# kan-bayashi/espnet

Hardware: AMD Instinct MI355X
Metric: frames/sec, 12L Conformer hybrid CTC/attention training step (B=32 T=1000 d=256 per GPU) (higher is better)
Workload: dtype f32

## Files before the change

### espnet_amd/_lib.py

```python
import ctypes as C
import os

import torch

_HERE = os.path.dirname(os.path.abspath(__file__))
LIB_PATH = os.path.join(_HERE, "csrc", "libespnet_amd_hip.so")


class EamdError(RuntimeError):
    pass


class GatherT(C.Structure):
    _fields_ = [("enabled", C.c_int32), ("C", C.c_int32), ("ntap", C.c_int32), ("Ho", C.c_int32),
                ("Wo", C.c_int32), ("Hin", C.c_int32), ("Win", C.c_int32), ("sh", C.c_int32),
                ("sw", C.c_int32), ("dh", C.c_int32 * 9), ("dw", C.c_int32 * 9)]


class RowMapT(C.Structure):
    _fields_ = [("enabled", C.c_int32), ("Ho", C.c_int32), ("Wo", C.c_int32), ("Hc", C.c_int32),
                ("Wc", C.c_int32), ("sh", C.c_int32), ("oh", C.c_int32), ("sw", C.c_int32),
                ("ow", C.c_int32)]


class RowStatsT(C.Structure):
    _fields_ = [("part", C.c_void_p), ("col", C.c_void_p), ("zcol", C.c_void_p), ("zfix", C.c_void_p),
                ("fix", C.c_int32), ("reserved", C.c_int32),
                ("rowc", C.c_void_p), ("gscale", C.c_void_p), ("scale", C.c_float), ("reserved2", C.c_int32)]


class GemmT(C.Structure):
    _fields_ = [("A", C.c_void_p), ("B", C.c_void_p), ("C", C.c_void_p), ("bias", C.c_void_p),
                ("aux", C.c_void_p), ("R", C.c_void_p), ("colsum", C.c_void_p),
                ("M", C.c_int32), ("N", C.c_int32), ("K", C.c_int32),
                ("transA", C.c_int32), ("transB", C.c_int32),
                ("lda", C.c_int64), ("ldb", C.c_int64), ("ldc", C.c_int64), ("ldaux", C.c_int64),
                ("ldr", C.c_int64),
                ("batch1", C.c_int32), ("batch2", C.c_int32),
                ("sA1", C.c_int64), ("sA2", C.c_int64), ("sB1", C.c_int64), ("sB2", C.c_int64),
                ("sC1", C.c_int64), ("sC2", C.c_int64),
                ("alpha", C.c_float), ("beta", C.c_float),
                ("a_act", C.c_int32), ("b_act", C.c_int32), ("epilogue", C.c_int32),
                ("splitk", C.c_int32), ("precision", C.c_int32), ("tile", C.c_int32),
                ("gather", GatherT), ("cmap", RowMapT),
                ("Cb", C.c_void_p), ("in_dtype", C.c_int32), ("aux_dtype", C.c_int32),
                ("drop_p", C.c_float), ("drop_salt", C.c_uint64), ("drop_step", C.c_void_p), ("Hb", C.c_void_p),
                ("h_act", C.c_int32),
                ("a_drop_p", C.c_float), ("b_drop_p", C.c_float), ("a_drop_salt", C.c_uint64), ("b_drop_salt", C.c_uint64),
                ("h_dtype", C.c_int32),
                ("stats", RowStatsT)]


class FfnT(C.Structure):
    _fields_ = [("x", C.c_void_p), ("w1", C.c_void_p), ("b1", C.c_void_p), ("w2", C.c_void_p), ("b2", C.c_void_p),
                ("R", C.c_void_p), ("out", C.c_void_p), ("f", C.c_void_p), ("h", C.c_void_p),
                ("M", C.c_int32), ("D", C.c_int32), ("F", C.c_int32), ("act", C.c_int32),
                ("alpha", C.c_float), ("p_in", C.c_float), ("salt_in", C.c_uint64), ("p_out", C.c_float),
                ("salt_out", C.c_uint64), ("drop_step", C.c_void_p), ("dtype", C.c_int32), ("hsplit", C.c_int32),
                ("ln_x", C.c_void_p), ("ln_w", C.c_void_p), ("ln_b", C.c_void_p), ("ln_mean", C.c_void_p),
                ("ln_rstd", C.c_void_p), ("ln_eps", C.c_float), ("reserved2", C.c_int32),
                ("lnb_x", C.c_void_p), ("lnb_gamma", C.c_void_p), ("lnb_mean", C.c_void_p), ("lnb_rstd", C.c_void_p),
                ("lnb_dres", C.c_void_p), ("lnb_ws", C.c_void_p), ("lnb_drop_out", C.c_void_p), ("lnb_drop_salt", C.c_uint64),
                ("lnb_drop_p", C.c_float), ("reserved3", C.c_int32)]


class RowProjT(C.Structure):
    _fields_ = [("a", C.c_void_p), ("lda", C.c_int64), ("w", C.c_void_p), ("bias", C.c_void_p), ("R", C.c_void_p),
                ("ldr", C.c_int64), ("out", C.c_void_p), ("ldo", C.c_int64),
                ("M", C.c_int32), ("K", C.c_int32), ("N", C.c_int32), ("a_act", C.c_int32),
                ("alpha", C.c_float), ("p_out", C.c_float), ("salt_out", C.c_uint64), ("drop_step", C.c_void_p),
                ("ln_x", C.c_void_p), ("ln_w", C.c_void_p), ("ln_b", C.c_void_p), ("ln_mean", C.c_void_p),
                ("ln_rstd", C.c_void_p), ("ln_eps", C.c_float), ("lnb_drop_p", C.c_float),
                ("a_scale", C.c_void_p), ("a_shift", C.c_void_p), ("a_out", C.c_void_p),
                ("lnb_x", C.c_void_p), ("lnb_gamma", C.c_void_p), ("lnb_mean", C.c_void_p), ("lnb_rstd", C.c_void_p),
                ("lnb_dres", C.c_void_p), ("lnb_ws", C.c_void_p), ("lnb_drop_out", C.c_void_p), ("lnb_drop_salt", C.c_uint64)]


class FfnPackT(C.Structure):
    _fields_ = [("w1", C.c_void_p), ("w2", C.c_void_p), ("fwd_first", C.c_void_p), ("fwd_second", C.c_void_p),
                ("bwd_first", C.c_void_p), ("bwd_second", C.c_void_p), ("D", C.c_int32), ("F", C.c_int32)]


class RowProjPackT(C.Structure):
    _fields_ = [("w", C.c_void_p), ("image", C.c_void_p), ("K", C.c_int32), ("N", C.c_int32), ("ldw", C.c_int32),
                ("trans", C.c_int32)]


class LstmSeqFwdT(C.Structure):
    _fields_ = [("gx", C.c_void_p), ("w_hh", C.c_void_p), ("b_hh", C.c_void_p), ("live", C.c_void_p),
                ("h_out", C.c_void_p), ("c_out", C.c_void_p), ("y", C.c_void_p), ("acts", C.c_void_p),
                ("reverse", C.c_int32), ("reserved", C.c_int32)]


class LstmSeqBwdT(C.Structure):
    _fields_ = [("dy", C.c_void_p), ("w_t", C.c_void_p), ("acts", C.c_void_p), ("c_out", C.c_void_p),
                ("live", C.c_void_p), ("dgates", C.c_void_p), ("reverse", C.c_int32), ("reserved", C.c_int32)]


_lib = None

SYMBOLS = [
    "eamd_abi_version", "eamd_gemm", "eamd_gemm_multi", "eamd_gemm_group_plan", "eamd_gemm_group_launch", "eamd_ffn_fwd", "eamd_ffn_bwd", "eamd_ffn_pack_f32", "eamd_ffn_pack_bf16", "eamd_ffn_pack_f32_multi", "eamd_rowproj", "eamd_rowproj_pack_f32", "eamd_rowproj_lnb_workspace", "eamd_layernorm_fwd", "eamd_layernorm_bwd_workspace", "eamd_layernorm_bwd_drop_f32", "eamd_layernorm_bwd", "eamd_layernorm_bwd_reduce", "eamd_attn_fwd", "eamd_attn_bwd_q", "eamd_attn_fwd_f32", "eamd_attn_bwd_q_f32", "eamd_attn_bwd_kv_f32", "eamd_attn_bwd_kv", "eamd_softmax_fwd",
    "eamd_softmax_bwd", "eamd_lsm_loss", "eamd_argmax_rows", "eamd_reduce_sum", "eamd_log_softmax_rows", "eamd_transducer_expand_rows", "eamd_topk_rows", "eamd_topk_rows_i32", "eamd_weighted_topk_rows", "eamd_beam_step", "eamd_beam_step_dyn", "eamd_decode_self_attn_dyn", "eamd_beam_slots_dyn", "eamd_ctc_prefix_psi_dyn", "eamd_ctc_prefix_state_dyn", "eamd_embed_pe_dyn", "eamd_copy_jobs", "eamd_embed_pe_ld", "eamd_linear_rows_f32", "eamd_linear_rows_ln_f32", "eamd_decode_self_attn", "eamd_beam_slots", "eamd_decode_src_attn", "eamd_decode_src_attn_group", "eamd_decode_src_attn_split", "eamd_decode_src_attn_split_workspace", "eamd_weighted_sum", "eamd_beam_select", "eamd_beam_finish",
    "eamd_axpby", "eamd_cast_bf16", "eamd_scale_dev", "eamd_act_fwd", "eamd_act_bwd", "eamd_glu_fwd", "eamd_glu_bwd",
    "eamd_add_bias2", "eamd_add_cast_bf16", "eamd_add_block_f32", "eamd_add_cast_colsum2", "eamd_add_colsum2_f32", "eamd_colsum", "eamd_embed_pe", "eamd_embed_bwd", "eamd_posenc", "eamd_posenc_scaled", "eamd_posenc_scaled_bwd", "eamd_permute4",
    "eamd_dropout", "eamd_rng_advance", "eamd_dwconv_fwd", "eamd_dwconv_glu_fwd", "eamd_dwconv_glu_bwd_x", "eamd_dwconv_glu_bwd_w", "eamd_dwconv_bwd_x", "eamd_dwconv_bwd_w", "eamd_bn_nslab",
    "eamd_bn_stats", "eamd_bn_finalize", "eamd_bn_apply", "eamd_bn_bwd", "eamd_bn_stats_bounded", "eamd_bn_bwd_bounded", "eamd_mask_time", "eamd_conv1_fwd", "eamd_conv1_bwd_w_workspace", "eamd_conv1_bwd_w",
    "eamd_conv2_weight_prep", "eamd_conv2_weight_grad", "eamd_add_sos_eos", "eamd_ctc_collapse",
    "eamd_ctc_workspace_bytes", "eamd_ctc_loss", "eamd_ctc_prefix_score", "eamd_ctc_prefix_score_batch", "eamd_ctc_prefix_psi", "eamd_ctc_prefix_state", "eamd_grad_norm", "eamd_sched_step", "eamd_adam_step", "eamd_adadelta_step", "eamd_add_gradient_noise",
    "eamd_specaug", "eamd_global_mvn", "eamd_utterance_mvn", "eamd_reflect_pad", "eamd_logmel", "eamd_unfold1d", "eamd_fold1d", "eamd_attloc_convmax_fwd", "eamd_attloc_convmax_bwd", "eamd_layernorm_bwd_drop",
    "eamd_lstm_cell_fwd", "eamd_lstm_cell_bwd", "eamd_lstm_step_fwd", "eamd_lstm_step_bwd", "eamd_lstm_seq_sync_bytes", "eamd_lstm_seq_fwd", "eamd_lstm_seq_bwd", "eamd_lstm_seq_status", "eamd_lstm_seq_status_merge", "eamd_gru_cell_fwd", "eamd_gru_cell_bwd", "eamd_maxpool2x2_fwd", "eamd_maxpool2x2_bwd", "eamd_mask_rows",
    "eamd_joint_fwd", "eamd_joint_bwd", "eamd_rnnt_workspace", "eamd_rnnt_loss", "eamd_rnnt_grad", "eamd_rnnt_node_stats", "eamd_rnnt_node_stats_part", "eamd_rnnt_row_coef", "eamd_rnnt_alpha_beta", "eamd_rnnt_node_grad",
    "eamd_conv3x3_c1_fwd", "eamd_conv3x3_c1_bwd_w_workspace", "eamd_conv3x3_c1_bwd_w", "eamd_attloc_fwd", "eamd_attloc_bwd_energy", "eamd_attloc_bwd_workspace", "eamd_attloc_bwd_energy_conv", "eamd_attloc_bwd_conv",
    "eamd_att_dot_energy_fwd", "eamd_att_dot_energy_bwd", "eamd_att_ctx_fwd", "eamd_att_ctx_bwd",
]


def lib():
    global _lib
    if _lib is None:
        if not os.path.exists(LIB_PATH):
            raise EamdError(
                f"{LIB_PATH} not found: build it with `python -c 'import __graft_entry__ as g; g.build()'` "
                "or `make -C espnet_amd/csrc` (there is no CPU fallback)")
        _lib = C.CDLL(LIB_PATH)
        _lib.eamd_ctc_workspace_bytes.restype = C.c_int64
        _lib.eamd_layernorm_bwd_workspace.restype = C.c_int64
        _lib.eamd_rnnt_workspace.restype = C.c_int64
        _lib.eamd_attloc_bwd_workspace.restype = C.c_int64
        _lib.eamd_conv1_bwd_w_workspace.restype = C.c_int64
        _lib.eamd_lstm_seq_sync_bytes.restype = C.c_int64
        _lib.eamd_conv3x3_c1_bwd_w_workspace.restype = C.c_int64
        for s in SYMBOLS:
            getattr(_lib, s)
    return _lib


_raw_stream = getattr(torch._C, "_cuda_getCurrentRawStream", None)
_cur_device = getattr(torch._C, "_cuda_getDevice", None)


def stream_ptr():
    if _raw_stream is not None and _cur_device is not None:
        return C.c_void_p(_raw_stream(_cur_device()))
    return C.c_void_p(torch.cuda.current_stream().cuda_stream)


EAMD_EUNSUPPORTED = -2


def check(rc, what):
    if rc != 0:
        raise EamdError(f"{what} failed with code {rc}")


def ptr(t, offset=0):
    if t is None:
        return None
    if not t.is_cuda:
        raise EamdError("espnet_amd kernels need GPU tensors (no CPU fallback in the product path)")
    if offset == 0:
        return C.c_void_p(t.data_ptr())
    return C.c_void_p(t.data_ptr() + offset * t.element_size())


def f32(t):
    if t.dtype != torch.float32:
        raise EamdError(f"expected float32 tensor, got {t.dtype}")
    return t
```

### espnet_amd/functional.py

```python
import math

import torch

from . import ops
from .ops import (ACT_NONE, ACT_RELU, ACT_SWISH, EPI_DACT_FACTOR, EPI_MUL_AUX, EPI_MUL_DSWISH, EPI_MUL_RELU_MASK, EPI_NONE,
                  EPI_RELU)


class GradSink:

    on_done = None
    on_use = None

    @staticmethod
    def use(params):
        if GradSink.on_use is not None and torch.is_grad_enabled():
            GradSink.on_use(params)
        return params

    def __init__(self, params):
        self.params = list(params)
        self.ret = [None] * len(self.params)

    def buf(self, i):
# ... 876 lines not shown
        gl = d = bmean = None
        nbt = getattr(running_mean, "_eamd_nbt", None)
        if FUSE_GLU_DWCONV:
            d = ops.dwconv_glu_fwd(a, wd.view(Cc, K), bd_, B, T, Cc, K,
                                   bn=(bn_eps, bn_momentum, running_mean, running_var, nbt) if (training and bound is None) else None)
            if d is not None and training and bound is None:
                d, bmean, brstd = d
        if d is None:
            gl = ops.glu_fwd(a, Cc)
            d = ops.dwconv_fwd(gl, wd.view(Cc, K), bd_, B, T, Cc, K)
        if training:
            if bmean is None:
                bmean, brstd = ops.bn_stats(d, M, Cc, bn_eps, bn_momentum, running_mean, running_var, nbt, bound=bound)
        else:
            bmean = running_mean
            brstd = ops.axpby(running_var, None, 1.0, 0.0)
            brstd = torch.rsqrt_(brstd.add_(bn_eps))
        e = ops.bn_apply(d, bmean, brstd, g, be, M, Cc, act, adt)
        ctx.rp = rp
        if rp is not None:
            out = ops.rowproj(e, rp[2], Cc, bias=b2, R=x2, drop=(p_out, s_out) if p_out > 0.0 else None)
        elif p_out > 0.0 and (ops.fast() or ops.f32_epilogue_drop()):
            out = ops.linear_fwd(e, ops.wshadow(w2).view(Cc, Cc), b2, R=x2, drop=(p_out, s_out))
        elif p_out > 0.0:
            br = ops.linear_fwd(e, ops.wshadow(w2).view(Cc, Cc), b2)
            out = ops.axpby(x2, ops.dropout(br, p_out, s_out), 1.0, 1.0)
        else:
            out = ops.linear_fwd(e, ops.wshadow(w2).view(Cc, Cc), b2, R=x2 if eps is not None else None)
        ctx.save_for_backward(x2, mean, rstd, xn, a, gl, d, bmean, brstd, e)
        ctx.pr = GradSink.use(params)
        ctx.cfg = (B, T, D, Cc, K, act, training, drop)
        ctx.bound = bound
        ctx.prev = _prev_drop(x)
        return _tag_out(out.view(B, T, D), p_out, s_out)

    @staticmethod
    def backward(ctx, dout):
        x2, mean, rstd, xn, a, gl, d, bmean, brstd, e = ctx.saved_tensors
        ln_w, ln_b, w1, b1, wd, bd_, g, be, w2, b2 = ctx.pr
        B, T, D, Cc, K, act, training, (p_out, s_out) = ctx.cfg
        M = B * T
        adt = ops.act_dtype()
        sink = GradSink(ctx.pr)
        do = dout.reshape(M, D).contiguous()
        dob, g_drop = _grad_operand(dout, do, p_out, s_out)
        rp = ctx.rp if g_drop is None else None
        ops.linear_bwd_w(dob, e, sink.buf(8).view(Cc, Cc), db=sink.buf(9), a_drop=g_drop)
        if rp is not None:
            de = ops.rowproj(dob, rp[3], Cc)
        else:
            de = ops.linear_bwd_x(dob, ops.wshadow(w2).view(Cc, Cc), a_drop=g_drop)
        dd = ops.bn_bwd(de, d, bmean, brstd, g, be, sink.buf(6), sink.buf(7), M, Cc, act, training, bound=ctx.bound)
        if gl is None:
            da = ops.dwconv_glu_bwd_x(dd, wd.view(Cc, K), a, B, T, Cc, K, adt)
            if ctx.bound is not None:
                ops.mask_time(da, T, ctx.bound[1])
            ops.dwconv_glu_bwd_w(dd, a, sink.buf(4).view(Cc, K), sink.buf(5), B, T, Cc, K)
        else:
            dgl = ops.dwconv_bwd_x(dd, wd.view(Cc, K), B, T, Cc, K)
            ops.dwconv_bwd_w(dd, gl, sink.buf(4).view(Cc, K), sink.buf(5), B, T, Cc, K)
            da = ops.glu_bwd(dgl, a, Cc, adt)
            if ctx.bound is not None:
                ops.mask_time(da, T, ctx.bound[1])
        ops.linear_bwd_w(da, xn, sink.buf(2).view(2 * Cc, D), db=sink.buf(3))
        if rp is not None and da.dtype == torch.float32:
            dx = _rp_ln_bwd(da, rp[1], x2, ln_w, mean, rstd, do, sink.buf(0), sink.buf(1), ctx.prev, (B, T, D))
        else:
            dxn = ops.linear_bwd_x(da, ops.wshadow(w1).view(2 * Cc, D))
            dx = _ln_bwd_out(dxn, x2, ln_w, mean, rstd, do, sink.buf(0), sink.buf(1), ctx.prev, (B, T, D))
        return (dx, None, None, None, None, None, None, None, None) + sink.results()


_TAPS_FWD = [(kh, kw) for kh in range(3) for kw in range(3)]
_CLASSES = [((0, 0), [(0, 0), (0, 2), (2, 0), (2, 2)]), ((0, 1), [(0, 1), (2, 1)]),
            ((1, 0), [(1, 0), (1, 2)]), ((1, 1), [(1, 1)])]


def _conv3s2_fwd(y_in, w, b, B, Hi, Wi, Cc, adt):
    Ho, Wo = (Hi - 3) // 2 + 1, (Wi - 3) // 2 + 1
    wf, wd = ops.conv2_weight_prep(w, adt)
    g = ops.make_gather(Cc, _TAPS_FWD, Ho, Wo, Hi, Wi, 2, 2)
    M = B * Ho * Wo
    y = torch.empty(M, Cc, device=y_in.device, dtype=adt)
    ops.gemm(y_in, wf, y, M, Cc, 9 * Cc, 9 * Cc, Cc, Cc, transB=1, bias=b, epilogue=EPI_RELU, gather=g)
    return y, wd, Ho, Wo


def _conv3s2_bwd(dy, y_in, wd, dw_buf, db_buf, B, Hi, Wi, Ho, Wo, Cc, adt):
    dev = dy.device
    M = B * Ho * Wo
    ops.colsum(dy, db_buf)
    dwf = torch.zeros(9 * Cc, Cc, device=dev, dtype=torch.float32)
    g = ops.make_gather(Cc, _TAPS_FWD, Ho, Wo, Hi, Wi, 2, 2)
    f32_big = (not ops.fast()) and Cc % 128 == 0
    tile = 128 if f32_big else 64
    ntile = (9 * Cc // tile) * ((Cc + tile - 1) // tile)
    want = 1024 if ops.fast() else 1008 if f32_big else 2304
    sk = max(2, min(64, (want + ntile - 1) // ntile, max(1, M // 256)))
    ops.gemm(y_in, dy, dwf, 9 * Cc, Cc, M, 9 * Cc, Cc, Cc, transA=1, transB=1, gather=g, splitk=sk, tile=tile)
    ops.conv2_weight_grad(dwf, dw_buf, Cc, Cc)
    dy_in = torch.empty(y_in.shape, device=dev, dtype=adt)
    q0, classes = 0, []
    for (ph, pw), taps in _CLASSES:
        Hc, Wc = (Hi - ph + 1) // 2, (Wi - pw + 1) // 2
        if Hc > 0 and Wc > 0:
            gt = ops.make_gather(Cc, [((ph - kh) // 2, (pw - kw) // 2) for kh, kw in taps], Hc, Wc, Ho, Wo, 1, 1)
            cm = ops.make_rowmap(Hc, Wc, Hi, Wi, 2, ph, 2, pw)
            nt = len(taps)
            ops.gemm(dy, wd, dy_in, B * Hc * Wc, Cc, nt * Cc, nt * Cc, Cc, Cc, transB=1, b_off=q0 * Cc * Cc,
                     gather=gt, cmap=cm, epilogue=EPI_MUL_RELU_MASK, aux=y_in, ldaux=Cc, defer=classes)
        q0 += len(taps)
    ops.gemm_multi(classes)
    return dy_in


def _taps(k):
    return [(kh, kw) for kh in range(k) for kw in range(k)]


def _conv_ks_fwd(y_in, w, b, B, Hi, Wi, Cc, adt, k, st):
    Ho, Wo = (Hi - k) // st + 1, (Wi - k) // st + 1
    KK = k * k
    wf = torch.empty(KK, Cc, Cc, device=y_in.device, dtype=torch.float32)
    ops.permute4(w.contiguous(), wf, (Cc, Cc, KK, 1), (1, Cc, Cc * Cc, 0))
    wd = torch.empty(KK, Cc, Cc, device=y_in.device, dtype=torch.float32)
    ops.permute4(w.contiguous(), wd, (Cc, Cc, KK, 1), (Cc, 1, Cc * Cc, 0))
    wf, wd = ops.to_act(wf), ops.to_act(wd)
    M = B * Ho * Wo
    y32 = torch.empty(M, Cc, device=y_in.device, dtype=torch.float32)
    taps = _taps(k)
    for t0 in range(0, KK, 9):
        ch = taps[t0:t0 + 9]
        g = ops.make_gather(Cc, ch, Ho, Wo, Hi, Wi, st, st)
        ops.gemm(y_in, wf, y32, M, Cc, len(ch) * Cc, len(ch) * Cc, Cc, Cc, transB=1, bias=b if t0 == 0 else None,
                 beta=0.0 if t0 == 0 else 1.0, gather=g, b_off=t0 * Cc * Cc)
    y = ops.dropout(y32, 0.0, 0, act=ACT_RELU, out_dtype=adt)
    return y, wd, Ho, Wo


def _conv_ks_bwd(dy, y_in, wd, dw_buf, db_buf, B, Hi, Wi, Ho, Wo, Cc, adt, k, st):
    dev = dy.device
    M = B * Ho * Wo
    KK = k * k
    taps = _taps(k)
    ops.colsum(dy, db_buf)
    dwf = torch.zeros(KK * Cc, Cc, device=dev, dtype=torch.float32)
    for t0 in range(0, KK, 9):
        ch = taps[t0:t0 + 9]
        g = ops.make_gather(Cc, ch, Ho, Wo, Hi, Wi, st, st)
        ntile = (len(ch) * Cc // 64) * ((Cc + 63) // 64)
        sk = max(2, min(64, (1024 + ntile - 1) // ntile, max(1, M // 256)))
        ops.gemm(y_in, dy, dwf, len(ch) * Cc, Cc, M, len(ch) * Cc, Cc, Cc, transA=1, transB=1, gather=g, splitk=sk, tile=64,
                 c_off=t0 * Cc * Cc)
    ops.permute4(dwf, dw_buf, (KK, Cc, Cc, 1), (1, KK, Cc * KK, 0), accumulate=True)
    dy_in = torch.empty(y_in.shape, device=dev, dtype=adt)
    order, classes = [], []
    for ph in range(st):
        for pw in range(st):
            ct = [(kh, kw) for kh in range(ph, k, st) for kw in range(pw, k, st)]
            classes.append(((ph, pw), ct))
            order += [kh * k + kw for kh, kw in ct]
    wd_cls = wd.index_select(0, torch.tensor(order, device=dev)).contiguous()
    q0, jobs = 0, []
    for (ph, pw), ct in classes:
        Hc, Wc = (Hi - ph + st - 1) // st, (Wi - pw + st - 1) // st
        if Hc > 0 and Wc > 0 and ct:
            gt = ops.make_gather(Cc, [((ph - kh) // st, (pw - kw) // st) for kh, kw in ct], Hc, Wc, Ho, Wo, 1, 1)
            cm = ops.make_rowmap(Hc, Wc, Hi, Wi, st, ph, st, pw)
            nt = len(ct)
            ops.gemm(dy, wd_cls, dy_in, B * Hc * Wc, Cc, nt * Cc, nt * Cc, Cc, Cc, transB=1, b_off=q0 * Cc * Cc,
                     gather=gt, cmap=cm, epilogue=EPI_MUL_RELU_MASK, aux=y_in, ldaux=Cc, defer=jobs)
        q0 += len(ct)
    ops.gemm_multi(jobs)
    return dy_in


class Conv2dSubsamplingFn(torch.autograd.Function):

    @staticmethod
    def forward(ctx, x, xscale, c1_w, c1_b, lin_w, lin_b, *convs):
        B, T, F = x.shape
        Cc = c1_w.shape[0]
        D = lin_w.shape[0]
        H1, W1 = (T - 3) // 2 + 1, (F - 3) // 2 + 1
# ... 174 lines not shown
```

### espnet_amd/ops.py

```python
import ctypes as C
import os
import math

import torch

from . import _lib
from ._lib import GatherT, GemmT, RowMapT, check, ptr, stream_ptr

ACT_NONE, ACT_RELU, ACT_SWISH = 0, 1, 2
EPI_NONE, EPI_RELU, EPI_SWISH, EPI_MUL_RELU_MASK, EPI_MUL_DSWISH, EPI_MUL_AUX, EPI_DACT_FACTOR, EPI_ROW_STATS, EPI_ROW_GRAD = 0, 1, 2, 3, 4, 5, 6, 7, 8

_PRECISIONS = {"fp32": 0, "bf16": 1}
_state = {"precision": 0}


def set_precision(name):
    if name not in _PRECISIONS:
        raise ValueError(f"precision must be one of {list(_PRECISIONS)}")
    _state["precision"] = _PRECISIONS[name]


def get_precision():
    return [k for k, v in _PRECISIONS.items() if v == _state["precision"]][0]

# ... 1450 lines not shown

def dwconv_glu_bwd_x(dy, w, a, B, T, Cc, K, out_dtype=torch.float32):
    da = torch.empty(a.shape, device=a.device, dtype=out_dtype)
    check(_lib.lib().eamd_dwconv_glu_bwd_x(ptr(dy), ptr(w), ptr(a), ptr(da), int(out_dtype == torch.bfloat16), B, T, Cc, K,
                                           stream_ptr()), "eamd_dwconv_glu_bwd_x")
    return da


def dwconv_glu_bwd_w(dy, a, dw, db, B, T, Cc, K):
    assert dw.numel() == Cc * K and (db is None or db.numel() == Cc)
    check(_lib.lib().eamd_dwconv_glu_bwd_w(ptr(dy), ptr(a), ptr(dw), ptr(db), B, T, Cc, K, stream_ptr()),
          "eamd_dwconv_glu_bwd_w")


def bn_stats(x, M, Cc, eps, momentum, running_mean, running_var, num_batches_tracked=None, bound=None):
    nslab = _lib.lib().eamd_bn_nslab(C.c_int64(M), Cc)
    ws = torch.empty(3 * Cc * nslab, device=x.device, dtype=torch.float32)
    mean = torch.empty(Cc, device=x.device, dtype=torch.float32)
    rstd = torch.empty(Cc, device=x.device, dtype=torch.float32)
    assert num_batches_tracked is None or (num_batches_tracked.dtype == torch.int64 and num_batches_tracked.is_cuda)
    if bound is not None:
        check(_lib.lib().eamd_bn_stats_bounded(ptr(x), ptr(ws), ptr(mean), ptr(rstd), ptr(running_mean), ptr(running_var),
                                               ptr(num_batches_tracked), C.c_int64(M), Cc, C.c_float(eps), C.c_float(momentum),
                                               int(bound[0]), ptr(bound[1]), stream_ptr()), "eamd_bn_stats_bounded")
        return mean, rstd
    check(_lib.lib().eamd_bn_stats(ptr(x), ptr(ws), ptr(mean), ptr(rstd), ptr(running_mean), ptr(running_var),
                                   ptr(num_batches_tracked), C.c_int64(M), Cc, C.c_float(eps), C.c_float(momentum), stream_ptr()),
          "eamd_bn_stats")
    return mean, rstd


def bn_apply(x, mean, rstd, gamma, beta, M, Cc, act, out_dtype=torch.float32):
    y = torch.empty(x.shape, device=x.device, dtype=out_dtype)
    check(_lib.lib().eamd_bn_apply(ptr(x), ptr(mean), ptr(rstd), ptr(gamma), ptr(beta), ptr(y), C.c_int64(M), Cc,
                                   act, 1 if out_dtype == torch.bfloat16 else 0, stream_ptr()), "eamd_bn_apply")
    return y


def bn_bwd(dy, x, mean, rstd, gamma, beta, dgamma, dbeta, M, Cc, act, training, bound=None):
    nslab = _lib.lib().eamd_bn_nslab(C.c_int64(M), Cc)
    ws = torch.empty((2 * nslab + 2) * Cc, device=x.device, dtype=torch.float32)
    dx = torch.empty_like(x)
    if bound is not None:
        check(_lib.lib().eamd_bn_bwd_bounded(ptr(dy), ptr(x), ptr(mean), ptr(rstd), ptr(gamma), ptr(beta), ptr(ws), ptr(dx),
                                             ptr(dgamma), ptr(dbeta), C.c_int64(M), Cc, act, int(training), int(bound[0]),
                                             ptr(bound[1]), stream_ptr()), "eamd_bn_bwd_bounded")
        return dx
    check(_lib.lib().eamd_bn_bwd(ptr(dy), ptr(x), ptr(mean), ptr(rstd), ptr(gamma), ptr(beta), ptr(ws), ptr(dx),
                                 ptr(dgamma), ptr(dbeta), C.c_int64(M), Cc, act, int(training), stream_ptr()),
          "eamd_bn_bwd")
    return dx


def conv1_fwd(x, w, bias, B, T, F, Cc, out_dtype=torch.float32):
    H, W = (T - 3) // 2 + 1, (F - 3) // 2 + 1
    assert x.numel() == B * T * F and w.numel() == Cc * 9
    y = torch.empty(B, H, W, Cc, device=x.device, dtype=out_dtype)
    check(_lib.lib().eamd_conv1_fwd(ptr(x), ptr(w), ptr(bias), ptr(y), B, T, F, Cc,
                                    1 if out_dtype == torch.bfloat16 else 0, stream_ptr()), "eamd_conv1_fwd")
    return y


def conv1_bwd_w(dy, x, dw, db, B, T, F, Cc):
    L = _lib.lib()
    ws = torch.empty(int(L.eamd_conv1_bwd_w_workspace(B, T, Cc)), device=x.device, dtype=torch.float32)
    check(L.eamd_conv1_bwd_w(ptr(dy), ptr(x), ptr(dw), ptr(db), ptr(ws), B, T, F, Cc,
                             1 if dy.dtype == torch.bfloat16 else 0, stream_ptr()), "eamd_conv1_bwd_w")


def conv2_weight_prep(w, out_dtype=torch.float32):
    Co, Ci = w.shape[0], w.shape[1]
    wf = torch.empty(9, Ci, Co, device=w.device, dtype=out_dtype)
    wd = torch.empty(9, Co, Ci, device=w.device, dtype=out_dtype)
    check(_lib.lib().eamd_conv2_weight_prep(ptr(w), ptr(wf), ptr(wd), Co, Ci,
                                            1 if out_dtype == torch.bfloat16 else 0, stream_ptr()),
          "eamd_conv2_weight_prep")
    return wf, wd


def conv2_weight_grad(dwf, dw, Co, Ci):
    check(_lib.lib().eamd_conv2_weight_grad(ptr(dwf), ptr(dw), Co, Ci, stream_ptr()), "eamd_conv2_weight_grad")


def permute4(src, dst, dims, dst_strides, accumulate=False):
    d0, d1, d2, d3 = dims
    s0, s1, s2, s3 = dst_strides
    assert src.numel() == d0 * d1 * d2 * d3
    assert (d0 - 1) * s0 + (d1 - 1) * s1 + (d2 - 1) * s2 + (d3 - 1) * s3 < dst.numel()
    check(_lib.lib().eamd_permute4(ptr(src), ptr(dst), d0, d1, d2, d3, C.c_int64(s0), C.c_int64(s1), C.c_int64(s2),
                                   C.c_int64(s3), int(accumulate), stream_ptr()), "eamd_permute4")


def add_sos_eos(ys_pad, sos, eos, ignore_id):
    B, L = ys_pad.shape
    assert ys_pad.dtype == torch.int64 and ys_pad.is_contiguous()
    ys_in = torch.empty(B, L + 1, device=ys_pad.device, dtype=torch.int64)
    ys_out = torch.empty(B, L + 1, device=ys_pad.device, dtype=torch.int64)
    olen = torch.empty(B, device=ys_pad.device, dtype=torch.int32)
    check(_lib.lib().eamd_add_sos_eos(ptr(ys_pad), ptr(ys_in), ptr(ys_out), ptr(olen), B, L, sos, eos, ignore_id,
                                      stream_ptr()), "eamd_add_sos_eos")
    return ys_in, ys_out, olen


def ctc_collapse(ids, hlens, blank):
    B, T = ids.shape
    assert ids.dtype == torch.int32 and ids.is_contiguous()
    out = torch.empty(B, T, device=ids.device, dtype=torch.int32)
    outlen = torch.empty(B, device=ids.device, dtype=torch.int32)
    check(_lib.lib().eamd_ctc_collapse(ptr(ids), ptr(hlens), ptr(out), ptr(outlen), B, T, blank, stream_ptr()),
          "eamd_ctc_collapse")
    return out, outlen


def ctc_loss(acts_btv, ys_pad, ilens, blank=0, ignore_id=-1, grad_scale=1.0, want_grad=True, time_major=False):
    if time_major:
        T, B, V = acts_btv.shape
        st, sb = B * V, V
    else:
        B, T, V = acts_btv.shape
        st, sb = V, T * V
    L = ys_pad.shape[1]
    assert acts_btv.is_contiguous() and ys_pad.is_contiguous() and ys_pad.dtype == torch.int64
    assert ilens.dtype == torch.int32 and ilens.numel() == B and ys_pad.shape[0] == B
    ws_bytes = _lib.lib().eamd_ctc_workspace_bytes(B, T, L)
    ws = torch.empty(ws_bytes, device=acts_btv.device, dtype=torch.uint8)
    nll = torch.empty(B, device=acts_btv.device, dtype=torch.float32)
    grad = torch.empty_like(acts_btv) if want_grad else None
    check(_lib.lib().eamd_ctc_loss(ptr(acts_btv), C.c_int64(st), C.c_int64(sb), ptr(ys_pad), ptr(ilens), ptr(nll),
                                   ptr(grad), C.c_int64(st), C.c_int64(sb), ptr(ws), B, T, V, L, blank, ignore_id,
                                   C.c_float(grad_scale), stream_ptr()), "eamd_ctc_loss")
    return nll, grad


def ctc_prefix_score(logp, r_prev, cand, last, olen, blank, eos):
    T, V = logp.shape
    nhyp, ncand = cand.shape
    assert r_prev.shape == (nhyp, T, 2) and cand.dtype == torch.int32 and logp.is_contiguous()
    psi = torch.empty(nhyp, ncand, device=logp.device, dtype=torch.float32)
    r_new = torch.empty(nhyp, ncand, T, 2, device=logp.device, dtype=torch.float32)
    check(_lib.lib().eamd_ctc_prefix_score(ptr(logp), ptr(r_prev.contiguous()), ptr(cand.contiguous()), ptr(last),
                                           ptr(olen), ptr(psi), ptr(r_new), nhyp, ncand, T, V, blank, eos,
                                           stream_ptr()), "eamd_ctc_prefix_score")
    return psi, r_new


def ctc_prefix_score_batch(logp, lens, per_utt, r_prev, cand, last, olen, blank, eos):
    U, Tmax, V = logp.shape
    nhyp, ncand = cand.shape
    assert nhyp == U * per_utt and r_prev.shape == (nhyp, Tmax, 2) and cand.dtype == torch.int32 and logp.is_contiguous()
    assert lens.dtype == torch.int32 and lens.numel() == U
    psi = torch.empty(nhyp, ncand, device=logp.device, dtype=torch.float32)
    r_new = torch.zeros(nhyp, ncand, Tmax, 2, device=logp.device, dtype=torch.float32)
    check(_lib.lib().eamd_ctc_prefix_score_batch(ptr(logp), ptr(lens), U, per_utt, ptr(r_prev.contiguous()), ptr(cand.contiguous()),
                                                 ptr(last), ptr(olen), ptr(psi), ptr(r_new), ncand, Tmax, V, blank, eos,
                                                 stream_ptr()), "eamd_ctc_prefix_score_batch")
    return psi, r_new


def ctc_prefix_psi(logp, lens, per_utt, r_prev, cand, last, olen, blank, eos, olen_dev=None):
    U, Tmax, V = logp.shape
    nhyp, ncand = cand.shape
    assert nhyp == U * per_utt and r_prev.shape == (nhyp, Tmax, 2) and cand.dtype == torch.int32 and logp.is_contiguous()
    psi = torch.empty(nhyp, ncand, device=logp.device, dtype=torch.float32)
    rc = _lib.lib().eamd_ctc_prefix_psi_dyn(ptr(logp), ptr(lens), U, per_utt, ptr(r_prev.contiguous()), ptr(cand.contiguous()), ptr(last),
                                            int(olen), ptr(olen_dev), ptr(psi), ncand, Tmax, V, blank, eos, stream_ptr())
    if rc == _lib.EAMD_EUNSUPPORTED:
# ... 608 lines not shown
```

### include/espnet_amd.h

```cpp
#ifndef ESPNET_AMD_H_
#define ESPNET_AMD_H_
#include <stdint.h>
#ifdef __cplusplus
extern "C" {
#endif

int eamd_abi_version(void);

typedef struct {
  int32_t enabled;
  int32_t C;
  int32_t ntap;
  int32_t Ho, Wo;
  int32_t Hin, Win;
  int32_t sh, sw;
  int32_t dh[9], dw[9];
} eamd_gather_t;

typedef struct {
  int32_t enabled;
  int32_t Ho, Wo;
  int32_t Hc, Wc;
  int32_t sh, oh, sw, ow;
} eamd_rowmap_t;
// ... 332 lines not shown
int eamd_lstm_seq_bwd(const eamd_lstm_seq_bwd_t* jobs, int njobs, int T, int B, int H, void* sync_ws, void* stream);
int eamd_lstm_seq_status(const void* sync_ws, void* stream);
int eamd_lstm_seq_status_merge(const void* sync_ws, void* sticky, void* stream);
int eamd_gru_cell_fwd(const float* gx, const float* gh, const float* h_prev, const uint8_t* live, float* h, float* y,
                      float* acts, int B, int H, void* stream);
int eamd_gru_cell_bwd(const float* dy, const float* dh, const float* acts, const float* h_prev, const uint8_t* live,
                      float* dgx, float* dgh, float* dh_direct, int B, int H, void* stream);
int eamd_maxpool2x2_fwd(const float* x, float* y, uint8_t* idx, int B, int H, int W, int C, void* stream);
int eamd_maxpool2x2_bwd(const float* dy, const uint8_t* idx, float* dx, int B, int H, int W, int C, void* stream);
int eamd_mask_rows(const float* x, const uint8_t* keep, float* y, int64_t rows, int D, void* stream);
int eamd_unfold1d(const void* x, void* col, int B, int T, int C, int k, int bf16, void* stream);
int eamd_fold1d(const float* dcol, float* dx, int B, int T, int C, int k, void* stream);
int eamd_conv3x3_c1_fwd(const float* x, const float* w, const float* bias, void* y, int B, int T, int F, int C,
                        int y_bf16, void* stream);
int64_t eamd_conv3x3_c1_bwd_w_workspace(int B, int T, int C);
int eamd_conv3x3_c1_bwd_w(const void* dy, const float* x, float* dw, float* db, float* workspace, int B, int T, int F,
                          int C, int dy_bf16, void* stream);
int eamd_attloc_fwd(const float* att_prev, const float* conv_w, const float* w_att, const float* pre_enc,
                    const float* dec_proj, const float* gvec, const float* gb, const int32_t* lens, const float* enc_h,
                    float scaling, float* e, float* th, float* conv, float* w, float* ctx, int B, int T, int A, int C,
                    int K, int R, int E, void* stream);
int eamd_attloc_bwd_energy(const float* dctx, const float* dw_ext, const float* w, const float* enc_h, const float* th,
                           const float* gvec, float scaling, float* de, float* d_enc_h, float* df, float* dgvec,
                           float* dgb, float* d_dec_proj, int B, int T, int A, int E, void* stream);
int64_t eamd_attloc_bwd_workspace(int B, int T, int A, int C);
int eamd_attloc_bwd_energy_conv(const float* dctx, const float* dw_ext, const float* w, const float* enc_h, const float* th,
                                const float* gvec, float scaling, const float* conv, const float* w_att, float* de,
                                float* d_enc_h, float* df, float* dconv, float* dgvec, float* dgb, float* d_dec_proj,
                                float* dw_att, float* workspace, int accumulate, int B, int T, int A, int C, int E,
                                void* stream);
int eamd_att_dot_energy_fwd(const float* k, const float* q, const int32_t* lens, float* e, int B, int T, int A,
                            void* stream);
int eamd_att_dot_energy_bwd(const float* de, const float* k, const float* q, float* dk, float* dq, int B, int T, int A,
                            void* stream);
int eamd_att_ctx_fwd(const float* e, const float* v, float scaling, float* w, float* ctx, int B, int T, int E,
                     void* stream);
int eamd_att_ctx_bwd(const float* dctx, const float* dw_ext, const float* w, const float* v, float scaling, float* de,
                     float* d_v, float* dsum, int B, int T, int E, void* stream);
int eamd_attloc_bwd_conv(const float* dconv, const float* conv_w, const float* att_prev, float* d_prev, float* dconv_w,
                         int B, int T, int C, int K, int R, void* stream);
int eamd_attloc_convmax_fwd(const float* att_prev, const float* conv_w, float* pooled, int32_t* idx, int B, int T, int C,
                            int K, void* stream);
int eamd_attloc_convmax_bwd(const float* dpool, const float* pooled, const int32_t* idx, const float* att_prev,
                            const float* conv_w, float* d_prev, float* dconv_w, int B, int T, int C, int K, void* stream);

int eamd_joint_fwd(const float* enc, const float* dec, float* out, void* out_bf16, int B, int T, int U, int J, int act,
                   void* stream);
int eamd_joint_bwd(const float* dh, const float* enc, const float* dec, float* d_enc, float* d_dec, int B, int T, int U,
                   int J, int act, void* stream);
int64_t eamd_rnnt_workspace(int B, int T, int U);
int eamd_rnnt_loss(const float* logits, const int32_t* labels, const int32_t* tlens, const int32_t* ulens,
                   float* workspace, float* loss, float* grad, int B, int T, int U, int V, int blank,
                   const float* gscale_dev, float scale, void* stream);
int eamd_rnnt_grad(const float* logits, const int32_t* labels, const int32_t* tlens, const int32_t* ulens,
                   const float* workspace, float* grad, int B, int T, int U, int V, int blank, const float* gscale_dev,
                   float scale, void* stream);
int eamd_rnnt_node_stats(const float* logits_rows, const int32_t* labels, float* workspace, int64_t node0, int64_t nrows,
                         int B, int T, int U, int V, int blank, void* stream);
int eamd_rnnt_alpha_beta(float* workspace, const int32_t* tlens, const int32_t* ulens, float* loss, int B, int T, int U,
                         void* stream);
int eamd_rnnt_node_stats_part(const float* part, const float* zlab, const float* zblank, float* workspace, int64_t node0,
                              int64_t nrows, int tiles_n, int B, int T, int U, void* stream);
int eamd_rnnt_row_coef(const int32_t* labels, const int32_t* tlens, const int32_t* ulens, const float* workspace, float* rowc,
                       int32_t* col, int64_t node0, int64_t nrows, int B, int T, int U, void* stream);
int eamd_rnnt_node_grad(const float* logits_rows, float* grad_rows, void* grad_rows_bf16, const int32_t* labels,
                        const int32_t* tlens, const int32_t* ulens, const float* workspace, int64_t node0, int64_t nrows,
                        int B, int T, int U, int V, int blank, const float* gscale_dev, float scale, void* stream);

int eamd_grad_norm(const float* g, int64_t n, float* workspace, float* gnorm_out, void* stream);
int eamd_sched_step(float* state, const float* gnorm, int mode, float base_lr, float factor, float dmodel,
                    float warmup, float beta1, float beta2, float max_norm, void* stream);
int eamd_adam_step(float* p, const float* g, float* m, float* v, void* p_bf16, int64_t n, const float* state,
                   float beta1, float beta2, float eps, float weight_decay, void* stream);
int eamd_adadelta_step(float* p, const float* g, float* square_avg, float* acc_delta, void* p_bf16, int64_t n,
                       const float* state, float rho, float weight_decay, void* stream);
int eamd_add_gradient_noise(float* g, int64_t n, float sigma, const uint64_t* step_dev, uint64_t salt, void* stream);

int eamd_add_sos_eos(const int64_t* ys_pad, int64_t* ys_in, int64_t* ys_out, int32_t* olen, int B, int L, int sos,
                     int eos, int ignore_id, void* stream);
int eamd_ctc_collapse(const int32_t* ids, const int32_t* hlens, int32_t* out, int32_t* outlen, int B, int T,
                      int blank, void* stream);
int eamd_conv2_weight_prep(const float* w, void* wf, void* wd, int Co, int Ci, int out_bf16, void* stream);
int eamd_conv2_weight_grad(const float* dwf, float* dw, int Co, int Ci, void* stream);

#ifdef __cplusplus
}
#endif
#endif
```

Before: 1.125 million.

## Add dedicated f32 MFMA kernels for stride-2 3x3 subsampling conv fwd and dx

```diff
diff --git a/espnet_amd/_lib.py b/espnet_amd/_lib.py
--- a/espnet_amd/_lib.py
+++ b/espnet_amd/_lib.py
@@ -106,7 +106,7 @@
     "eamd_add_bias2", "eamd_add_cast_bf16", "eamd_add_block_f32", "eamd_add_cast_colsum2", "eamd_add_colsum2_f32", "eamd_colsum", "eamd_embed_pe", "eamd_embed_bwd", "eamd_posenc", "eamd_posenc_scaled", "eamd_posenc_scaled_bwd", "eamd_permute4",
     "eamd_dropout", "eamd_rng_advance", "eamd_dwconv_fwd", "eamd_dwconv_glu_fwd", "eamd_dwconv_glu_bwd_x", "eamd_dwconv_glu_bwd_w", "eamd_dwconv_bwd_x", "eamd_dwconv_bwd_w", "eamd_bn_nslab",
     "eamd_bn_stats", "eamd_bn_finalize", "eamd_bn_apply", "eamd_bn_bwd", "eamd_bn_stats_bounded", "eamd_bn_bwd_bounded", "eamd_mask_time", "eamd_conv1_fwd", "eamd_conv1_bwd_w_workspace", "eamd_conv1_bwd_w",
-    "eamd_conv2_weight_prep", "eamd_conv2_weight_grad", "eamd_add_sos_eos", "eamd_ctc_collapse",
+    "eamd_conv2_weight_prep", "eamd_conv2_weight_grad", "eamd_conv3s2_f32_fwd", "eamd_conv3s2_f32_bwd_x", "eamd_add_sos_eos", "eamd_ctc_collapse",
     "eamd_ctc_workspace_bytes", "eamd_ctc_loss", "eamd_ctc_prefix_score", "eamd_ctc_prefix_score_batch", "eamd_ctc_prefix_psi", "eamd_ctc_prefix_state", "eamd_grad_norm", "eamd_sched_step", "eamd_adam_step", "eamd_adadelta_step", "eamd_add_gradient_noise",
     "eamd_specaug", "eamd_global_mvn", "eamd_utterance_mvn", "eamd_reflect_pad", "eamd_logmel", "eamd_unfold1d", "eamd_fold1d", "eamd_attloc_convmax_fwd", "eamd_attloc_convmax_bwd", "eamd_layernorm_bwd_drop",
     "eamd_lstm_cell_fwd", "eamd_lstm_cell_bwd", "eamd_lstm_step_fwd", "eamd_lstm_step_bwd", "eamd_lstm_seq_sync_bytes", "eamd_lstm_seq_fwd", "eamd_lstm_seq_bwd", "eamd_lstm_seq_status", "eamd_lstm_seq_status_merge", "eamd_gru_cell_fwd", "eamd_gru_cell_bwd", "eamd_maxpool2x2_fwd", "eamd_maxpool2x2_bwd", "eamd_mask_rows",
diff --git a/espnet_amd/csrc/conv3s2_f32.hip b/espnet_amd/csrc/conv3s2_f32.hip
--- /dev/null
+++ b/espnet_amd/csrc/conv3s2_f32.hip
@@ -0,0 +1,310 @@
+#include "common.h"
+#include "../../include/espnet_amd.h"
+
+namespace {
+
+constexpr int CT = 512;
+constexpr int CBM = 128, CBK = 32;
+constexpr int CLDA = CBK + 4;
+constexpr int QD = 8, NS = CBK / QD, EQ = QD / 4;
+
+template <int BN>
+struct SmemC {
+  static constexpr int LDB = BN + 8;
+  static constexpr int LDC = BN + 4;
+  static constexpr int OPS = 2 * CBM * CLDA + 2 * CBK * LDB;
+  static constexpr int CTS = 64 * LDC;
+  float ab[OPS > CTS ? OPS : CTS];
+  __device__ float* a(int buf) { return ab + buf * CBM * CLDA; }
+  __device__ float* b(int buf) { return ab + 2 * CBM * CLDA + buf * CBK * LDB; }
+};
+
+struct ConvArgs {
+  const float* x;
+  const float* w;
+  const float* bias;
+  const float* aux;
+  float* y;
+  int Hi, Wi, Ho, Wo, C;
+  int rows;
+  int tiles_n;
+  int ntile;
+};
+
+constexpr unsigned kDhNeg = (1u << 2) | (1u << 3) | (1u << 5);
+constexpr unsigned kDwNeg = (1u << 1) | (1u << 3) | (1u << 7);
+
+template <int BN, bool DX>
+__device__ __forceinline__ void conv_tile(SmemC<BN>& sm, const ConvArgs& p, const int m0, const int n0, const int q0,
+                                          const int nkt, const int ph, const int pw) {
+  constexpr int WN = BN / 4, NTL = WN / 16, MT = 4;
+  constexpr int CPR_B = BN / 4, RPP_B = CT / CPR_B, NCB = CBK / RPP_B;
+  static_assert(NCB == 2 || NCB == 4, "B staging is written out for 2 or 4 chunks per thread");
+  constexpr int NCA = CBM * CBK / 4 / CT;
+  constexpr int LDB = SmemC<BN>::LDB;
+  const int t = threadIdx.x, lane = t & 63, wave = t >> 6;
+  const int wm = wave >> 2, wn = wave & 3;
+  const int C = p.C;
+  const float* __restrict__ X = p.x;
+  const float* __restrict__ W = p.w;
+
+  int a_r[NCA];
+  const int a_c = t & 7;
+  int a_base[NCA], a_i[NCA], a_j[NCA];
+#pragma unroll
+  for (int i = 0; i < NCA; ++i) {
+    a_r[i] = (t >> 3) + 64 * i;
+    const int m = min(m0 + a_r[i], p.rows - 1);
+    if constexpr (!DX) {
+      const int j = m % p.Wo, tt = m / p.Wo, ii = tt % p.Ho, b = tt / p.Ho;
+      a_base[i] = (b * p.Hi + 2 * ii) * p.Wi + 2 * j;
+      a_i[i] = 0; a_j[i] = 0;
+    } else {
+      const int Wc = p.Wo + 1, Hc = p.Ho + 1;
+      const int j = m % Wc, tt = m / Wc, ii = tt % Hc, b = tt / Hc;
+      a_base[i] = (b * p.Ho + ii) * p.Wo + j;
+      a_i[i] = ii; a_j[i] = j;
+    }
+  }
+  const int b_r = t / CPR_B, b_c = t % CPR_B;
+  const float* __restrict__ Wt = W + (long)q0 * C * C + n0 + b_c * 4;
+
+  f32x4 ra[NCA], rb[NCB];
+  bool aok[NCA];
+  auto load_tile = [&](int kt) __attribute__((always_inline)) {
+    const int k0 = kt * CBK;
+    const int tap = k0 / C, c0 = k0 - tap * C;
+#pragma unroll
+    for (int i = 0; i < NCA; ++i) {
+      long off;
+      if constexpr (!DX) {
+        const int kh = tap / 3, kw = tap - 3 * (tap / 3);
+        off = (long)(a_base[i] + kh * p.Wi + kw) * C;
+        aok[i] = true;
+      } else {
+        const int q = q0 + tap;
+        const int dh = -(int)((kDhNeg >> q) & 1u), dw = -(int)((kDwNeg >> q) & 1u);
+        const int ii = a_i[i] + dh, jj = a_j[i] + dw;
+        aok[i] = ii >= 0 && ii < p.Ho && jj >= 0 && jj < p.Wo;
+        off = aok[i] ? (long)(a_base[i] + dh * p.Wo + dw) * C : 0L;
+      }
+      ra[i] = *reinterpret_cast<const f32x4*>(X + off + c0 + a_c * 4);
+    }
+    const float* wk = Wt + (long)(k0 + b_r) * C;
+    const long wstep = (long)RPP_B * C;
+    rb[0] = *reinterpret_cast<const f32x4*>(wk);
+    rb[1] = *reinterpret_cast<const f32x4*>(wk + wstep);
+    if constexpr (NCB == 4) {
+      rb[2] = *reinterpret_cast<const f32x4*>(wk + 2 * wstep);
+      rb[3] = *reinterpret_cast<const f32x4*>(wk + 3 * wstep);
+    }
+  };
+  auto store_tile = [&](int buf) __attribute__((always_inline)) {
+    float* la = sm.a(buf);
+    float* lb = sm.b(buf);
+#pragma unroll
+    for (int i = 0; i < NCA; ++i) {
+      f32x4 v = ra[i];
+      if constexpr (DX) {
+        if (!aok[i]) v = (f32x4){0.f, 0.f, 0.f, 0.f};
+      }
+      *reinterpret_cast<f32x4*>(&la[a_r[i] * CLDA + a_c * 4]) = v;
+    }
+#pragma unroll
+    for (int i = 0; i < NCB; ++i) *reinterpret_cast<f32x4*>(&lb[(b_r + RPP_B * i) * LDB + b_c * 4]) = rb[i];
+  };
+
+  f32x4 acc[MT][NTL];
+#pragma unroll
+  for (int i = 0; i < MT; ++i)
+#pragma unroll
+    for (int j = 0; j < NTL; ++j) acc[i][j] = (f32x4){0.f, 0.f, 0.f, 0.f};
+
+  const int fr = lane & 15, fq = lane >> 4;
+  auto read_frags = [&](int buf, int q, float (&af)[MT][EQ], float (&bfr)[NTL][EQ]) __attribute__((always_inline)) {
+    const float* la = sm.a(buf);
+    const float* lb = sm.b(buf);
+#pragma unroll
+    for (int i = 0; i < MT; ++i) {
+      const float2 v = *reinterpret_cast<const float2*>(&la[(wm * 64 + i * 16 + fr) * CLDA + q * QD + fq * EQ]);
+      af[i][0] = v.x; af[i][1] = v.y;
+    }
+#pragma unroll
+    for (int j = 0; j < NTL; ++j)
+#pragma unroll
+      for (int e = 0; e < EQ; ++e) bfr[j][e] = lb[(q * QD + fq * EQ + e) * LDB + wn * WN + j * 16 + fr];
+  };
+  auto mfma_set = [&](const float (&af)[MT][EQ], const float (&bfr)[NTL][EQ]) __attribute__((always_inline)) {
+#pragma unroll
+    for (int e = 0; e < EQ; ++e)
+#pragma unroll
+      for (int i = 0; i < MT; ++i)
+#pragma unroll
+        for (int j = 0; j < NTL; ++j)
+          acc[i][j] = __builtin_amdgcn_mfma_f32_16x16x4f32(af[i][e], bfr[j][e], acc[i][j], 0, 0, 0);
+  };
+
+  load_tile(0);
+  store_tile(0);
+  __syncthreads();
+  float fa[2][MT][EQ], fb[2][NTL][EQ];
+  read_frags(0, 0, fa[0], fb[0]);
+  for (int it = 0; it < nkt; ++it) {
+    const int buf = it & 1;
+    load_tile(min(it + 1, nkt - 1));
+#pragma unroll
+    for (int q = 0; q < NS; ++q) {
+      if (q + 1 < NS) {
+        read_frags(buf, q + 1, fa[(q + 1) & 1], fb[(q + 1) & 1]);
+      } else {
+        __builtin_amdgcn_sched_barrier(0);
+        __syncthreads();
+        read_frags(buf ^ 1, 0, fa[0], fb[0]);
+#pragma unroll
+        for (int e = 0; e < EQ; ++e) {
+#pragma unroll
+          for (int i = 0; i < MT; ++i) asm volatile("" : "+v"(fa[q & 1][i][e]));
+#pragma unroll
+          for (int j = 0; j < NTL; ++j) asm volatile("" : "+v"(fb[q & 1][j][e]));
+        }
+      }
+      __builtin_amdgcn_sched_barrier(0);
+      if (q == NS - 2) {
+        store_tile(buf ^ 1);
+        __builtin_amdgcn_sched_barrier(0);
+      }
+      mfma_set(fa[q & 1], fb[q & 1]);
+    }
+  }
+  __syncthreads();
+
+  constexpr int LDC = SmemC<BN>::LDC;
+  constexpr int RPP_C = CT / CPR_B;
+  float* cl = sm.ab;
+  const int c4 = t % CPR_B;
+  const int n = n0 + c4 * 4;
+  float4 bv = make_float4(0.f, 0.f, 0.f, 0.f);
+  if constexpr (!DX) bv = *reinterpret_cast<const float4*>(p.bias + n);
+#pragma unroll
+  for (int h = 0; h < 2; ++h) {
+    if (wm == h) {
+#pragma unroll
+      for (int i = 0; i < MT; ++i)
+#pragma unroll
+        for (int j = 0; j < NTL; ++j)
+#pragma unroll
+          for (int r = 0; r < 4; ++r) cl[(i * 16 + fq * 4 + r) * LDC + wn * WN + j * 16 + fr] = acc[i][j][r];
+    }
+    __syncthreads();
+#pragma unroll
+    for (int rr = t / CPR_B; rr < 64; rr += RPP_C) {
+      const int m = m0 + h * 64 + rr;
+      if (m >= p.rows) continue;
+      float4 v = *reinterpret_cast<const float4*>(&cl[rr * LDC + c4 * 4]);
+      long orow;
+      if constexpr (!DX) {
+        orow = m;
+        v.x += bv.x; v.y += bv.y; v.z += bv.z; v.w += bv.w;
+        v = make_float4(v.x > 0.f ? v.x : 0.f, v.y > 0.f ? v.y : 0.f, v.z > 0.f ? v.z : 0.f, v.w > 0.f ? v.w : 0.f);
+      } else {
+        const int Wc = p.Wo + 1, Hc = p.Ho + 1;
+        const int j = m % Wc, tt = m / Wc, ii = tt % Hc, b = tt / Hc;
+        const int hi = 2 * ii + ph, wi = 2 * j + pw;
+        if (hi >= p.Hi || wi >= p.Wi) continue;
+        orow = ((long)b * p.Hi + hi) * p.Wi + wi;
+        const float4 ax = *reinterpret_cast<const float4*>(p.aux + orow * C + n);
+        v = make_float4(ax.x > 0.f ? v.x : 0.f, ax.y > 0.f ? v.y : 0.f, ax.z > 0.f ? v.z : 0.f, ax.w > 0.f ? v.w : 0.f);
+      }
+      *reinterpret_cast<float4*>(p.y + orow * C + n) = v;
+    }
+    __syncthreads();
+  }
+}
+
+__device__ __forceinline__ int xcd_tile(int id, int ntile) {
+  const int q = ntile >> 3, r = ntile & 7, xcd = id & 7, j = id >> 3;
+  return (xcd < r ? xcd * (q + 1) : r * (q + 1) + (xcd - r) * q) + j;
+}
+
+template <int BN>
+__global__ __launch_bounds__(CT, 1) void conv3s2_f32_fwd_kernel(const ConvArgs p) {
+  extern __shared__ __attribute__((aligned(16))) char smem_raw[];
+  SmemC<BN>& sm = *reinterpret_cast<SmemC<BN>*>(smem_raw);
+  const int tile = xcd_tile(blockIdx.x, p.ntile);
+  const int tm = tile / p.tiles_n, tn = tile - tm * p.tiles_n;
+  conv_tile<BN, false>(sm, p, tm * CBM, tn * BN, 0, 9 * p.C / CBK, 0, 0);
+}
+
+template <int BN>
+__global__ __launch_bounds__(CT, 1) void conv3s2_f32_dx_kernel(const ConvArgs p) {
+  extern __shared__ __attribute__((aligned(16))) char smem_raw[];
+  SmemC<BN>& sm = *reinterpret_cast<SmemC<BN>*>(smem_raw);
+  const int tile = xcd_tile(blockIdx.x, p.ntile);
+  const int tm = tile / p.tiles_n, tn = tile - tm * p.tiles_n;
+  const int kc = p.C / CBK;
+  const int s = ((int)blockIdx.x >> 3) & 3;
+  for (int c = 0; c < 4; ++c) {
+    const int cls = (c + s) & 3;
+    const int q0 = cls == 0 ? 0 : cls == 1 ? 4 : cls == 2 ? 6 : 8;
+    const int nt = cls == 0 ? 4 : cls == 3 ? 1 : 2;
+    conv_tile<BN, true>(sm, p, tm * CBM, tn * BN, q0, nt * kc, cls >> 1, cls & 1);
+  }
+}
+
+bool al16(const void* q) { return (reinterpret_cast<uintptr_t>(q) & 15) == 0; }
+
+template <int BN, bool DX>
+int launch(const ConvArgs& p, hipStream_t stream) {
+  constexpr size_t smem = sizeof(SmemC<BN>);
+  const void* fn = DX ? reinterpret_cast<const void*>(&conv3s2_f32_dx_kernel<BN>)
+                      : reinterpret_cast<const void*>(&conv3s2_f32_fwd_kernel<BN>);
+  static const hipError_t attr_err = hipFuncSetAttribute(fn, hipFuncAttributeMaxDynamicSharedMemorySize, (int)smem);
+  if (attr_err != hipSuccess) return (int)attr_err;
+  if constexpr (DX) hipLaunchKernelGGL((conv3s2_f32_dx_kernel<BN>), dim3(p.ntile), dim3(CT), smem, stream, p);
+  else hipLaunchKernelGGL((conv3s2_f32_fwd_kernel<BN>), dim3(p.ntile), dim3(CT), smem, stream, p);
+  EAMD_LAUNCH_CHECK();
+  return EAMD_OK;
+}
+
+int make_args(ConvArgs& p, int B, int Hi, int Wi, int C, bool dx) {
+  if (B <= 0 || C <= 0 || C % 128 != 0 || Hi < 3 || Wi < 3) return EAMD_EUNSUPPORTED;
+  p.Hi = Hi; p.Wi = Wi; p.C = C;
+  p.Ho = (Hi - 3) / 2 + 1; p.Wo = (Wi - 3) / 2 + 1;
+  const long pix_in = (long)B * Hi * Wi;
+  const long rows = dx ? (long)B * (p.Ho + 1) * (p.Wo + 1) : (long)B * p.Ho * p.Wo;
+  if (pix_in >= (1L << 31) || rows >= (1L << 31)) return EAMD_EUNSUPPORTED;
+  p.rows = (int)rows;
+  p.tiles_n = C % 256 == 0 ? C / 256 : C / 128;
+  const long nt = (rows + CBM - 1) / CBM * p.tiles_n;
+  if (nt >= (1L << 31)) return EAMD_EUNSUPPORTED;
+  p.ntile = (int)nt;
+  return EAMD_OK;
+}
+
+}
+
+extern "C" {
+
+int eamd_conv3s2_f32_fwd(const float* x, const float* wf, const float* bias, float* y, int B, int Hi, int Wi, int C,
+                         void* stream) {
+  if (!x || !wf || !bias || !y) return EAMD_EINVAL;
+  ConvArgs p{};
+  const int rc = make_args(p, B, Hi, Wi, C, false);
+  if (rc != EAMD_OK) return rc;
+  if (!al16(x) || !al16(wf) || !al16(bias) || !al16(y)) return EAMD_EUNSUPPORTED;
+  p.x = x; p.w = wf; p.bias = bias; p.aux = nullptr; p.y = y;
+  return C % 256 == 0 ? launch<256, false>(p, (hipStream_t)stream) : launch<128, false>(p, (hipStream_t)stream);
+}
+
+int eamd_conv3s2_f32_bwd_x(const float* dy, const float* wd, const float* y_in, float* dy_in, int B, int Hi, int Wi, int C,
+                           void* stream) {
+  if (!dy || !wd || !y_in || !dy_in) return EAMD_EINVAL;
+  ConvArgs p{};
+  const int rc = make_args(p, B, Hi, Wi, C, true);
+  if (rc != EAMD_OK) return rc;
+  if (!al16(dy) || !al16(wd) || !al16(y_in) || !al16(dy_in)) return EAMD_EUNSUPPORTED;
+  p.x = dy; p.w = wd; p.bias = nullptr; p.aux = y_in; p.y = dy_in;
+  return C % 256 == 0 ? launch<256, true>(p, (hipStream_t)stream) : launch<128, true>(p, (hipStream_t)stream);
+}
+
+}
diff --git a/espnet_amd/functional.py b/espnet_amd/functional.py
--- a/espnet_amd/functional.py
+++ b/espnet_amd/functional.py
@@ -982,6 +982,8 @@
     g = ops.make_gather(Cc, _TAPS_FWD, Ho, Wo, Hi, Wi, 2, 2)
     M = B * Ho * Wo
     y = torch.empty(M, Cc, device=y_in.device, dtype=adt)
+    if adt == torch.float32 and Cc % 128 == 0 and ops.conv3s2_f32_fwd(y_in, wf, b, y, B, Hi, Wi, Cc):
+        return y, wd, Ho, Wo
     ops.gemm(y_in, wf, y, M, Cc, 9 * Cc, 9 * Cc, Cc, Cc, transB=1, bias=b, epilogue=EPI_RELU, gather=g)
     return y, wd, Ho, Wo
 
@@ -1000,6 +1002,8 @@
     ops.gemm(y_in, dy, dwf, 9 * Cc, Cc, M, 9 * Cc, Cc, Cc, transA=1, transB=1, gather=g, splitk=sk, tile=tile)
     ops.conv2_weight_grad(dwf, dw_buf, Cc, Cc)
     dy_in = torch.empty(y_in.shape, device=dev, dtype=adt)
+    if adt == torch.float32 and Cc % 128 == 0 and ops.conv3s2_f32_bwd_x(dy, wd, y_in, dy_in, B, Hi, Wi, Cc):
+        return dy_in
     q0, classes = 0, []
     for (ph, pw), taps in _CLASSES:
         Hc, Wc = (Hi - ph + 1) // 2, (Wi - pw + 1) // 2
diff --git a/espnet_amd/ops.py b/espnet_amd/ops.py
--- a/espnet_amd/ops.py
+++ b/espnet_amd/ops.py
@@ -1556,6 +1556,26 @@
     check(_lib.lib().eamd_conv2_weight_grad(ptr(dwf), ptr(dw), Co, Ci, stream_ptr()), "eamd_conv2_weight_grad")
 
 
+def conv3s2_f32_fwd(x, wf, bias, y, B, Hi, Wi, Cc):
+    assert x.dtype == wf.dtype == y.dtype == torch.float32 and x.numel() == B * Hi * Wi * Cc and wf.numel() == 9 * Cc * Cc
+    assert y.numel() == B * ((Hi - 3) // 2 + 1) * ((Wi - 3) // 2 + 1) * Cc and bias.numel() == Cc
+    rc = _lib.lib().eamd_conv3s2_f32_fwd(ptr(x), ptr(wf), ptr(bias), ptr(y), B, Hi, Wi, Cc, stream_ptr())
+    if rc == _lib.EAMD_EUNSUPPORTED:
+        return False
+    check(rc, "eamd_conv3s2_f32_fwd")
+    return True
+
+
+def conv3s2_f32_bwd_x(dy, wd, y_in, dy_in, B, Hi, Wi, Cc):
+    assert dy.dtype == wd.dtype == y_in.dtype == dy_in.dtype == torch.float32 and wd.numel() == 9 * Cc * Cc
+    assert dy.numel() == B * ((Hi - 3) // 2 + 1) * ((Wi - 3) // 2 + 1) * Cc and y_in.numel() == dy_in.numel() == B * Hi * Wi * Cc
+    rc = _lib.lib().eamd_conv3s2_f32_bwd_x(ptr(dy), ptr(wd), ptr(y_in), ptr(dy_in), B, Hi, Wi, Cc, stream_ptr())
+    if rc == _lib.EAMD_EUNSUPPORTED:
+        return False
+    check(rc, "eamd_conv3s2_f32_bwd_x")
+    return True
+
+
 def permute4(src, dst, dims, dst_strides, accumulate=False):
     d0, d1, d2, d3 = dims
     s0, s1, s2, s3 = dst_strides
diff --git a/include/espnet_amd.h b/include/espnet_amd.h
--- a/include/espnet_amd.h
+++ b/include/espnet_amd.h
@@ -438,6 +438,10 @@
                       int blank, void* stream);
 int eamd_conv2_weight_prep(const float* w, void* wf, void* wd, int Co, int Ci, int out_bf16, void* stream);
 int eamd_conv2_weight_grad(const float* dwf, float* dw, int Co, int Ci, void* stream);
+int eamd_conv3s2_f32_fwd(const float* x, const float* wf, const float* bias, float* y, int B, int Hi, int Wi, int C,
+                         void* stream);
+int eamd_conv3s2_f32_bwd_x(const float* dy, const float* wd, const float* y_in, float* dy_in, int B, int Hi, int Wi, int C,
+                           void* stream);
 
 #ifdef __cplusplus
 }
```

New measurement: 1.127 million, median of 6. Within noise of the previous version (+0.2%).
